# bytedance/ps-lite

Hardware: AMD Instinct MI355X
Metric: push+pull GB/s per worker + p50 round-trip µs, 1 MB & 64 MB, at 1/2/4/8 GPUs (higher is better)
Workload: dtype fp32; 1 GPU; model=dense push+pull (ps-lite test_benchmark PUSH_PULL), global_batch=128, seq_len=67108864, parallelism=byteps-joint x1 (worker+server per GPU), mode=dense, msg_bytes=67108864, batch_keys=False, overlap=True, op=assign

## Files before the change

### csrc/customer.cc

```cpp
#include "customer.h"

#include <chrono>

#include "postoffice.h"

namespace xps {

Customer::Customer(int app_id, int customer_id, RecvHandle handle, Postoffice* po)
    : app_id_(app_id), customer_id_(customer_id), handle_(std::move(handle)), po_(po) {
  po_->AddCustomer(this);
  thread_ = std::thread([this] { Receiving(); });
}

Customer::~Customer() {
  po_->RemoveCustomer(this);
  Message term;
  term.meta.control.cmd = Control::TERMINATE;
  queue_.Push(std::move(term));
  if (thread_.joinable()) thread_.join();
}

int Customer::NewRequest(int recver) {
  std::lock_guard<std::mutex> lk(mu_);
  int expected = recver >= 8 ? 1 : static_cast<int>(po_->GetNodeIDs(recver).size());
  tracker_.emplace_back();
  tracker_.back().expected = expected;
  return static_cast<int>(tracker_.size()) - 1;
}

Customer::Slot* Customer::GetSlot(int ts) {
  std::lock_guard<std::mutex> lk(mu_);
  XPS_CHECK_LT(static_cast<size_t>(ts), tracker_.size());
  return &tracker_[ts];
}

void Customer::WaitRequest(int ts) {
  Slot* s = GetSlot(ts);
  auto deadline = std::chrono::steady_clock::now() + std::chrono::microseconds(150);
  while (s->received.load(std::memory_order_acquire) < s->expected) {
    if (std::chrono::steady_clock::now() >= deadline) break;
  }
  if (s->received.load(std::memory_order_acquire) >= s->expected) return;
  static const int timeout_s = Environment::Get()->GetInt("XPS_WAIT_TIMEOUT_S", 0);
  std::unique_lock<std::mutex> lk(mu_);
  auto done = [s] { return s->received.load(std::memory_order_acquire) >= s->expected; };
  if (timeout_s <= 0) {
    cv_.wait(lk, done);
    return;
  }
  if (!cv_.wait_for(lk, std::chrono::seconds(timeout_s), done)) {
    XPS_LOG(Fatal) << "request ts=" << ts << " (app " << app_id_ << ") got "
                   << s->received.load() << "/" << s->expected << " responses after "
                   << timeout_s << " s — responder dead? (XPS_WAIT_TIMEOUT_S)";
  }
}

bool Customer::IsFinished(int ts) {
  Slot* s = GetSlot(ts);
  return s->received.load(std::memory_order_acquire) >= s->expected;
}

int Customer::NumResponse(int ts) {
  return GetSlot(ts)->received.load(std::memory_order_acquire);
}

void Customer::AddResponse(int ts, int num) {
  Slot* s = GetSlot(ts);
  int got = s->received.fetch_add(num, std::memory_order_acq_rel) + num;
  if (got >= s->expected) {
    std::lock_guard<std::mutex> lk(mu_);
    cv_.notify_all();
  }
}

thread_local int g_in_handler = 0;

bool InCustomerHandler() { return g_in_handler > 0; }

void Customer::RunHandle(Message& msg) {
  g_in_handler++;
  handle_(msg);
  g_in_handler--;
  if (!msg.meta.request) AddResponse(msg.meta.timestamp, 1);
}

void Customer::ProcessInline(Message& msg) {
  XPS_STAGE(customer_process);
  std::lock_guard<std::mutex> lk(handle_mu_);
  RunHandle(msg);
}

void Customer::Receiving() {
  while (true) {
    Message msg;
    queue_.WaitAndPop(&msg);
    if (msg.meta.control.cmd == Control::TERMINATE) break;
    std::lock_guard<std::mutex> lk(handle_mu_);
    RunHandle(msg);
  }
}

}
```

### csrc/customer.h

```cpp
#pragma once

#include <atomic>
#include <condition_variable>
#include <deque>
#include <functional>
#include <mutex>
#include <thread>
#include <utility>

#include "message.h"
#include "queue.h"

namespace xps {

class Postoffice;

bool InCustomerHandler();

class Customer {
 public:
  using RecvHandle = std::function<void(const Message&)>;

  Customer(int app_id, int customer_id, RecvHandle handle, Postoffice* po);
  ~Customer();
  Customer(const Customer&) = delete;

  int app_id() const { return app_id_; }
  int customer_id() const { return customer_id_; }

  int NewRequest(int recver);
  void WaitRequest(int ts);
  int NumResponse(int ts);
  void AddResponse(int ts, int num = 1);
  bool IsFinished(int ts);

  void Accept(Message msg) { queue_.Push(std::move(msg)); }

  void ProcessInline(Message& msg);

 private:
  struct Slot {
    int expected = 0;
    std::atomic<int> received{0};
  };

  void Receiving();
  void RunHandle(Message& msg);
  Slot* GetSlot(int ts);

  int app_id_;
  int customer_id_;
  RecvHandle handle_;
  Postoffice* po_;
  ThreadsafeQueue<Message> queue_;
  std::thread thread_;
  std::mutex handle_mu_;
  std::mutex mu_;
  std::condition_variable cv_;
  std::deque<Slot> tracker_;
};

}
```

### csrc/gpu_plane.cc

```cpp
#include "gpu_plane.h"

#include <fcntl.h>
#include <hip/hip_runtime.h>
#include <semaphore.h>
#include <sys/prctl.h>
#include <time.h>
#include <unistd.h>

#include <cstring>

#include "hip_pool.h"
#include "host_par.h"
#include "host_pool.h"
#include "kernels.h"
#include "postoffice.h"
#include "wire.h"

namespace xps {

static const size_t kInlineMax = 4096;

#define XPS_HIP_CHECK(cmd)                                                            \
  do {                                                                                \
    hipError_t e_ = (cmd);                                                            \
    XPS_CHECK(e_ == hipSuccess) << "HIP error: " << hipGetErrorString(e_) << " in " #cmd; \
  } while (0)

std::atomic<uint64_t> g_zero_copy_recv{0};
std::atomic<uint64_t> g_fused_assign{0};

bool FusedAssignEnabled() {
  static const bool on = Environment::Get()->GetInt("XPS_FUSED_ASSIGN", 1) != 0;
  return on;
}

std::atomic<uint64_t> g_fused_launches{0};

bool CoalesceEnabled() {
  static const bool on = Environment::Get()->GetInt("XPS_COALESCE", 1) != 0;
  return on;
}

namespace {
struct CoTicket {
  const void* plane = nullptr;
  int peer = 0;
  std::shared_ptr<void> cev;
};
thread_local CoTicket t_co_ticket;

int64_t NowUs() {
  struct timespec ts;
  clock_gettime(CLOCK_MONOTONIC, &ts);
  return static_cast<int64_t>(ts.tv_sec) * 1000000 + ts.tv_nsec / 1000;
}
const int64_t kHoldQuietUs = 2000;
const size_t kCoBusyBytes = 16u << 20;

std::mutex g_map_mu;
struct HandleKey {
  char h[kIpcHandleBytes];
  bool operator==(const HandleKey& o) const { return memcmp(h, o.h, kIpcHandleBytes) == 0; }
};
struct HandleHash {
  size_t operator()(const HandleKey& k) const {
    size_t v = 1469598103934665603ull;
    for (char c : k.h) {
      v ^= static_cast<unsigned char>(c);
      v *= 1099511628211ull;
    }
    return v;
  }
};
std::unordered_map<HandleKey, void*, HandleHash> g_mapped;

class IpcOpenLock {
 public:
  IpcOpenLock() {
    sem_ = sem_open("/xps_ipc_open_lock", O_CREAT, 0600, 1);
  }
  void Lock() {
    if (sem_ == SEM_FAILED) return;
    struct timespec ts;
    clock_gettime(CLOCK_REALTIME, &ts);
    ts.tv_sec += 60;
    if (sem_timedwait(sem_, &ts) != 0) {
      XPS_LOG(Warning) << "ipc-open lock timeout; proceeding unlocked";
      timed_out_ = true;
    }
  }
  void Unlock() {
    if (sem_ != SEM_FAILED && !timed_out_) sem_post(sem_);
    timed_out_ = false;
  }

 private:
  sem_t* sem_ = SEM_FAILED;
  bool timed_out_ = false;
};
IpcOpenLock g_ipc_lock;
}

GpuPlane::GpuPlane(Postoffice* po, int device) : po_(po), device_(device) {
  my_host_hash_ = HostHash();
  inline_deliver_ = Environment::Get()->GetInt("XPS_INLINE_HANDLER", 1) != 0;
  lanes_ = Environment::Get()->GetInt("XPS_STREAMS_PER_PEER", 2);
  if (lanes_ < 1) lanes_ = 1;
  if (lanes_ > 2) lanes_ = 2;
  co_hold_ = Environment::Get()->GetInt("XPS_COALESCE_HOLD", 0) != 0;
  int cap_mb = Environment::Get()->GetInt("XPS_COALESCE_CAP_MB", 1024);
  co_byte_cap_ = static_cast<size_t>(cap_mb < 1 ? 1 : cap_mb) << 20;
}

GpuPlane::~GpuPlane() { Stop(); }

void GpuPlane::FillSelf(Node* self) {
  static std::once_flag gc_once;
  std::call_once(gc_once, [] { HostShmPool::GcStaleSegments(); });
  self->dev_id = device_;
  auto* pool = HbmPool::Get();
  if (device_ >= 0 && pool->initialized()) {
    self->pool_capacity = pool->capacity();
    self->pool_slab_bytes = pool->slab_bytes();
    self->pool_handles.resize(pool->slab_count());
    for (size_t i = 0; i < pool->slab_count(); ++i) {
      memcpy(self->pool_handles[i].data(), pool->slab_handle(i), kIpcHandleBytes);
    }
  }
  auto* hpool = HostShmPool::Get();
  hpool->Init(self->shm_uid);
  self->host_pool_uid = hpool->uid();
  self->host_pool_capacity = hpool->capacity();
  if (!started_) {
    auto* env = Environment::Get();
    if (!env->GetInt("XPS_PROBE_NO_RING", 0)) {
      XPS_CHECK(in_ring_.Create(self->shm_uid)) << "cannot create shm ring";
    }
    started_ = true;
    if (!env->GetInt("XPS_PROBE_NO_POLL", 0)) {
      poll_running_ = true;
      poll_thread_ = std::thread([this] { RingPollLoop(); });
    }
    if (device_ >= 0 && !env->GetInt("XPS_PROBE_NO_COMP", 0)) {
      comp_thread_ = std::thread([this] { CompletionLoop(); });
    }
  }
}

void GpuPlane::Stop() {
  if (stop_.exchange(true)) return;
  PrintStageStats(device_ >= 0 ? "gpu plane" : "host plane");
  if (poll_thread_.joinable()) poll_thread_.join();
  if (comp_thread_.joinable()) comp_thread_.join();
  {
    std::lock_guard<std::mutex> lk(local_mu_);
    for (auto& lm : local_q_) po_->van()->Deliver(std::move(lm.first));
    local_q_.clear();
  }
  if (device_ >= 0) {
    std::vector<Peer*> all;
    {
      std::shared_lock<std::shared_timed_mutex> lk(peers_mu_);
      for (auto& kv : peers_) all.push_back(kv.second.get());
    }
// ... 187 lines not shown
          hipError_t e2 = hipMemcpy(probe, base, sizeof(probe), hipMemcpyDeviceToHost);
          if (e2 != hipSuccess) {
            XPS_LOG(Warning) << "peer " << p->node.id << " slab " << i
                             << " mapped but unreadable (" << hipGetErrorString(e2)
                             << ") — peer stays on the TCP path";
            base = nullptr;
          }
        }
        g_mapped[key] = base;
      }
    }
    if (!base) {
      std::lock_guard<std::mutex> lk(p->mu);
      p->slab_bases.clear();
      return false;
    }
    bases.push_back(base);
  }
  std::lock_guard<std::mutex> lk(p->mu);
  p->slab_bases = std::move(bases);
  return !p->slab_bases.empty();
}

char* GpuPlane::ResolvePeer(Peer* p, uint64_t global_off, uint64_t len) {
  if (!ImportPeerSlabs(p)) return nullptr;
  uint64_t slab_bytes = p->node.pool_slab_bytes;
  if (slab_bytes == 0) return nullptr;
  size_t idx = static_cast<size_t>(global_off / slab_bytes);
  uint64_t local = global_off % slab_bytes;
  std::lock_guard<std::mutex> lk(p->mu);
  if (idx >= p->slab_bases.size() || len > slab_bytes - local) {
    XPS_LOG(Warning) << "peer offset out of bounds: off=" << global_off << " len=" << len
                     << " slab=" << idx;
    return nullptr;
  }
  return static_cast<char*>(p->slab_bases[idx]) + local;
}

hipStream_t GpuPlane::StreamLane(int node_id, int lane) {
  if (lane >= lanes_) lane = lanes_ - 1;
  Peer* p = GetPeer(node_id);
  if (lane == 0) CoFlush(p);
  return RawLane(p, lane);
}

bool GpuPlane::LanesSplit(int node_id) {
  return lanes_ >= 2 && GetPeer(node_id)->node.dev_id != device_;
}


void GpuPlane::CoLaunchLocked(Peer* p) {
  Coalescer& co = p->co;
  if (co.n == 0) return;
  hipStream_t stream = RawLane(p, 0);
  XPS_HIP_CHECK(hipSetDevice(device_));
  if (co.n == 1) {
    const kern::Seg2& s = co.segs[0];
    kern::DenseAssign2(s.dst0, s.dst1, s.src, s.nbytes, stream);
  } else {
    kern::BatchedAssign2(co.segs, co.n, stream);
  }
  g_fused_launches.fetch_add(1, std::memory_order_relaxed);
  hipEvent_t ev = GetEvent();
  XPS_HIP_CHECK(hipEventRecord(ev, stream));
  co.open->bytes = co.bytes;
  co.open->ev.store(ev, std::memory_order_release);
  co.inflight.push_back(std::move(co.open));
  co.open.reset();
  co.n = 0;
  co.bytes = 0;
  co.n_open.store(0, std::memory_order_release);
}

bool GpuPlane::CoBusyLocked(Peer* p) {
  CoPruneLocked(p);
  size_t bytes = 0;
  for (auto& f : p->co.inflight) bytes += f->bytes;
  return p->co.inflight.size() >= 2 && bytes >= kCoBusyBytes;
}

void GpuPlane::CoPruneLocked(Peer* p) {
  auto& fl = p->co.inflight;
  while (!fl.empty()) {
    CoEvent* f = fl.front().get();
    if (!f->done.load(std::memory_order_acquire) &&
        hipEventQuery(f->ev.load(std::memory_order_acquire)) != hipSuccess) {
      break;
    }
    fl.pop_front();
  }
}

void GpuPlane::CoFlush(Peer* p) {
  if (p->co.n_open.load(std::memory_order_acquire) == 0) return;
  std::lock_guard<std::mutex> lk(p->co.mu);
  CoLaunchLocked(p);
}

std::shared_ptr<GpuPlane::CoEvent> GpuPlane::CoAppend(Peer* p, const kern::Seg2& seg) {
  if (!CoalesceEnabled()) return nullptr;
  Coalescer& co = p->co;
  std::lock_guard<std::mutex> lk(co.mu);
  kern::Admit a = kern::CoalesceAdmit(co.segs, co.n, seg);
  if (a != kern::Admit::kAdmit) CoLaunchLocked(p);
  if (a == kern::Admit::kReject) return nullptr;
  if (!co.open) co.open = std::make_shared<CoEvent>(this);
  std::shared_ptr<CoEvent> cev = co.open;
  co.segs[co.n++] = seg;
  co.bytes += seg.nbytes;
  co.n_open.store(co.n, std::memory_order_release);
  if (co.n >= kern::kMaxBatch || co.bytes >= co_byte_cap_) {
    CoLaunchLocked(p);
  } else if (co_hold_) {
    co.last_append_us = NowUs();
  } else {
    if (!CoBusyLocked(p)) CoLaunchLocked(p);
  }
  return cev;
}

bool GpuPlane::CoFrontUnlaunched(Peer* p, const std::shared_ptr<CoEvent>& cev) {
  Coalescer& co = p->co;
  std::lock_guard<std::mutex> lk(co.mu);
  if (co.open != cev) return true;
  if (co_hold_ && NowUs() - co.last_append_us < kHoldQuietUs) return false;
  CoLaunchLocked(p);
  return true;
}

void GpuPlane::CoRetired(Peer* p) {
  Coalescer& co = p->co;
  std::lock_guard<std::mutex> lk(co.mu);
  bool busy = CoBusyLocked(p);
  if (!co_hold_ && !busy) CoLaunchLocked(p);
}

bool GpuPlane::CoalesceAppend(int peer_id, const kern::Seg2& seg) {
  if (device_ < 0) return false;
  std::shared_ptr<CoEvent> cev = CoAppend(GetPeer(peer_id), seg);
  if (!cev) return false;
  t_co_ticket.plane = this;
  t_co_ticket.peer = peer_id;
  t_co_ticket.cev = std::move(cev);
  return true;
}

std::shared_ptr<GpuPlane::CoEvent> GpuPlane::TakeTicket(int peer_id) {
  if (!t_co_ticket.cev || t_co_ticket.plane != this || t_co_ticket.peer != peer_id) {
    return nullptr;
  }
  auto cev = std::static_pointer_cast<CoEvent>(t_co_ticket.cev);
  t_co_ticket.cev.reset();
  return cev;
}

void GpuPlane::CoalesceEnd(int peer_id) {
  if (!t_co_ticket.cev) return;
  t_co_ticket.cev.reset();
  CoFlush(GetPeer(peer_id));
}

hipStream_t GpuPlane::RawLane(Peer* p, int lane) {
  hipStream_t s = p->streams[lane].load(std::memory_order_acquire);
  if (s) return s;
  std::lock_guard<std::mutex> lk(p->mu);
  s = p->streams[lane].load(std::memory_order_relaxed);
  if (!s) {
    XPS_HIP_CHECK(hipSetDevice(device_));
    XPS_HIP_CHECK(hipStreamCreateWithFlags(&s, hipStreamNonBlocking));
    p->streams[lane].store(s, std::memory_order_release);
  }
  return s;
}

hipStream_t GpuPlane::StreamForPeer(int node_id) { return StreamLane(node_id, 0); }

hipStream_t GpuPlane::PullStreamForPeer(int node_id) {
  Peer* p = GetPeer(node_id);
  if (lanes_ < 2 || p->node.dev_id == device_) return StreamLane(node_id, 0);
  CoFlush(p);
  return StreamLane(node_id, 1);
}

std::vector<std::tuple<int, int64_t, int64_t>> GpuPlane::PeerBytes() {
  std::vector<std::tuple<int, int64_t, int64_t>> out;
  std::shared_lock<std::shared_timed_mutex> lk(peers_mu_);
  for (auto& kv : peers_) {
    int64_t tx = kv.second->tx_bytes.load(std::memory_order_relaxed);
    int64_t rx = kv.second->rx_bytes.load(std::memory_order_relaxed);
    if (tx || rx) out.emplace_back(kv.first, tx, rx);
  }
  return out;
// ... 137 lines not shown
bool GpuPlane::LocalPullRead(int peer_id, void* dst, uint64_t entry_off, size_t len,
                             Message resp) {
  if (device_ < 0 || !started_ || stop_.load()) return false;
  Peer* p = GetPeer(peer_id);
  char* src = ResolvePeer(p, entry_off, len);
  if (!src) return false;
  XPS_STAGE(local_pull_read);
  hipStream_t stream;
  if (Postoffice* elpo = LocalPeer(p)) {
    auto* rplane = dynamic_cast<GpuPlane*>(elpo->van() ? elpo->van()->plane() : nullptr);
    if (!rplane) return false;
    static const bool queue_req = Environment::Get()->GetInt("XPS_LOCAL_QUEUE_REQ", 0) != 0;
    if (!inline_deliver_ || queue_req) return false;
    stream = rplane->StreamForPeer(po_->node_id());
  } else {
    stream = StreamForPeer(peer_id);
  }
  XPS_HIP_CHECK(hipSetDevice(device_));
  kern::DenseAssign(dst, src, len, stream);
  g_zero_copy_recv.fetch_add(1, std::memory_order_relaxed);
  hipEvent_t ev = GetEvent();
  XPS_HIP_CHECK(hipEventRecord(ev, stream));
  int64_t bytes = static_cast<int64_t>(len) + 64;
  {
    std::lock_guard<std::mutex> lk(pend_mu_);
    pending_[peer_id].push_back(Pending{ev, peer_id, std::string(), std::move(resp), Message(),
                                        bytes, po_});
  }
  pending_count_.fetch_add(1);
  p->rx_bytes.fetch_add(bytes, std::memory_order_relaxed);
  return true;
}

bool GpuPlane::EntryPushPull(Message& msg, Peer* p, int64_t* bytes_out) {
  if (!FusedAssignEnabled()) return false;
  if (!(msg.meta.option & kOptPullAddr) || (msg.meta.option & kOptHostAddr)) return false;
  static const bool local_one_sided =
      Environment::Get()->GetInt("XPS_LOCAL_ONE_SIDED", 0) != 0;
  Postoffice* elpo = LocalPeer(p);
  GpuPlane* rplane =
      elpo ? dynamic_cast<GpuPlane*>(elpo->van() ? elpo->van()->plane() : nullptr) : nullptr;
  bool can = elpo ? (local_one_sided && rplane != nullptr) : EnsureRing(p);
  if (!can) return false;
  SArray<char> vals = msg.data[1];
  size_t len = vals.size();
  if (len == 0) return false;
  char* entry = ResolvePeer(p, msg.meta.entry_addr, len);
  char* dst = static_cast<char*>(HbmPool::Get()->PtrOf(msg.meta.addr, len));
  if (!entry || !dst || !kern::Disjoint3(entry, dst, vals.data(), len)) return false;
  XPS_STAGE(entry_push_pull);
  std::shared_ptr<CoEvent> cev;
  static const bool co_one_sided =
      Environment::Get()->GetInt("XPS_COALESCE_ONE_SIDED", 0) != 0;
  if (!elpo && co_one_sided) cev = CoAppend(p, kern::Seg2{entry, dst, vals.data(), len});
  hipStream_t stream = nullptr;
  if (!cev) {
    stream = elpo ? rplane->StreamForPeer(po_->node_id()) : StreamForPeer(p->node.id);
    XPS_HIP_CHECK(hipSetDevice(device_));
    kern::DenseAssign2(entry, dst, vals.data(), len, stream);
    g_fused_launches.fetch_add(1, std::memory_order_relaxed);
  }
  g_fused_assign.fetch_add(1, std::memory_order_relaxed);
  g_zero_copy_recv.fetch_add(1, std::memory_order_relaxed);
  Message meta_msg;
  meta_msg.meta = msg.meta;
  meta_msg.meta.option |= kOptInPlace;
  meta_msg.meta.val_len = static_cast<int64_t>(len);
  meta_msg.meta.data_type.clear();
  for (size_t i = 0; i < msg.data.size(); ++i) {
    if (i == 1 || msg.data[i].on_device()) continue;
    meta_msg.data.push_back(msg.data[i]);
    meta_msg.meta.data_type.push_back(msg.meta.data_type[i]);
  }
  int64_t bytes = 64 + static_cast<int64_t>(len);
  Message keepalive;
  keepalive.data.push_back(vals);
  std::string payload;
  if (!elpo) {
    std::vector<char> br(meta_msg.data.size(), 0);
    XPS_CHECK(Serialize(meta_msg, br, &payload));
  }
  hipEvent_t ev = nullptr;
  if (!cev) {
    ev = GetEvent();
    XPS_HIP_CHECK(hipEventRecord(ev, stream));
  }
  {
    std::lock_guard<std::mutex> lk(pend_mu_);
    pending_[p->node.id].push_back(Pending{ev, p->node.id, std::move(payload),
                                           std::move(meta_msg), std::move(keepalive), bytes,
                                           elpo, std::move(cev)});
  }
  pending_count_.fetch_add(1);
  p->tx_bytes.fetch_add(bytes, std::memory_order_relaxed);
  *bytes_out = bytes;
  return true;
}

void GpuPlane::EnqueueLocal(Message msg, int64_t bytes) {
  {
    std::lock_guard<std::mutex> lk(local_mu_);
    local_q_.emplace_back(std::move(msg), bytes);
  }
  local_count_.fetch_add(1, std::memory_order_release);
}

int64_t GpuPlane::SendLocal(Message& msg, Peer* p, Postoffice* lpo) {
// ... 263 lines not shown
    if (msg.data[i].on_device()) {
      by_ref[i] = 1;
      ref_bytes += msg.data[i].size();
      if (i == 1) msg.meta.option |= kOptValsByRef;
    } else if (msg.data[i].size() > kInlineMax) {
      by_ref[i] = 2;
      ref_bytes += msg.data[i].size();
    }
  }
  std::string payload;
  if (!Serialize(msg, by_ref, &payload)) {
    if (response && device_ >= 0) (void)hipStreamSynchronize(StreamForPeer(peer_node.id));
    return -1;
  }
  int64_t bytes = static_cast<int64_t>(payload.size()) + ref_bytes;
  bool kernel_less_ack = KernelLessAck(msg);
  if (response && device_ >= 0 && !kernel_less_ack) {
    hipStream_t stream = (msg.meta.option & kOptPullLane) ? PullStreamForPeer(peer_node.id)
                                                          : StreamForPeer(peer_node.id);
    Message resend = msg;
    DeferSendInternal(p, peer_node.id, stream, std::move(resend), Message(), std::move(payload),
                      bytes);
  } else {
    auto ring = RingOf(p);
    if (!ring || !ring->Push(payload.data(), static_cast<uint32_t>(payload.size()))) return -1;
    XPS_VLOG(3) << "plane send done -> " << peer_node.id;
  }
  p->tx_bytes.fetch_add(bytes, std::memory_order_relaxed);
  return bytes;
}

void GpuPlane::DeferSendInternal(Peer* p, int peer_id, hipStream_t stream, Message resend,
                                 Message keepalive, std::string payload, int64_t bytes) {
  XPS_STAGE(defer_queue);
  XPS_CHECK_GE(device_, 0) << "deferred sends are a GPU-plane feature";
  hipEvent_t ev = GetEvent();
  XPS_HIP_CHECK(hipSetDevice(device_));
  XPS_HIP_CHECK(hipEventRecord(ev, stream));
  {
    std::lock_guard<std::mutex> lk(pend_mu_);
    pending_[peer_id].push_back(Pending{ev, peer_id, std::move(payload), std::move(resend),
                                        std::move(keepalive), bytes});
  }
  pending_count_.fetch_add(1);
  XPS_VLOG(3) << "deferred send queued -> " << peer_id;
}

void GpuPlane::CompletionLoop() {
  XPS_HIP_CHECK(hipSetDevice(device_));
  prctl(PR_SET_TIMERSLACK, 1000);
  const int kSpin = Environment::Get()->GetInt("XPS_POLL_SPIN", 200000);
  int idle = 0;
  std::vector<int> ids;
  while (!stop_.load()) {
    bool did = false;
    if (pending_count_.load(std::memory_order_acquire) > 0) {
      ids.clear();
      {
        std::lock_guard<std::mutex> lk(pend_mu_);
        for (auto& kv : pending_) {
          if (!kv.second.empty()) ids.push_back(kv.first);
        }
      }
      for (int id : ids) {
        while (!stop_.load()) {
          hipEvent_t front_ev = nullptr;
          std::shared_ptr<CoEvent> cev;
          {
            std::lock_guard<std::mutex> lk(pend_mu_);
            auto& dq = pending_[id];
            if (dq.empty()) break;
            front_ev = dq.front().ev;
            cev = dq.front().cev;
          }
          bool retired = false;
          if (cev) {
            front_ev = cev->ev.load(std::memory_order_acquire);
            if (!front_ev) {
              if (!CoFrontUnlaunched(GetPeer(id), cev)) break;
              continue;
            }
          }
          if (!cev || !cev->done.load(std::memory_order_acquire)) {
            hipError_t e = hipEventQuery(front_ev);
            if (e == hipErrorNotReady) break;
            XPS_CHECK(e == hipSuccess) << "hipEventQuery: " << hipGetErrorString(e);
            if (cev) {
              cev->done.store(true, std::memory_order_release);
              retired = true;
            }
          }
          XPS_STAGE(defer_release);
          if (retired) CoRetired(GetPeer(id));
          Pending front;
          {
            std::lock_guard<std::mutex> lk(pend_mu_);
            auto& dq = pending_[id];
            front = std::move(dq.front());
            dq.pop_front();
          }
          pending_count_.fetch_sub(1);
          if (front.local_po) {
            DeliverLocal(front.local_po, front.resend, front.bytes);
            if (front.ev) PutEvent(front.ev);
            did = true;
            continue;
          }
          Peer* peer = GetPeer(front.peer_id);
          auto ring = peer ? RingOf(peer) : nullptr;
          bool sent = ring && ring->Push(front.payload.data(),
                                         static_cast<uint32_t>(front.payload.size()));
          if (sent) {
            XPS_VLOG(3) << "deferred send done -> " << front.peer_id;
          } else {
            XPS_LOG(Warning) << "deferred plane send failed -> " << front.peer_id
                             << "; falling back to TCP";
            if (po_->van()->SendOverTcp(front.resend, front.peer_id) < 0) {
              XPS_LOG(Warning) << "TCP fallback to " << front.peer_id
                               << " failed too (peer dead?)";
            }
          }
          if (front.ev) PutEvent(front.ev);
          did = true;
        }
      }
    }
    if (did) {
      idle = 0;
    } else if (++idle > kSpin) {
      usleep(20);
    }
  }
}

void GpuPlane::RingPollLoop() {
  if (device_ >= 0) XPS_HIP_CHECK(hipSetDevice(device_));
  prctl(PR_SET_TIMERSLACK, 1000);
  const int kSpin = Environment::Get()->GetInt("XPS_POLL_SPIN", 200000);
  std::vector<char> buf(ShmRing::MaxPayload());
  int idle = 0;
  std::deque<std::pair<Message, int64_t>> local;
  while (!stop_.load()) {
    if (local_count_.load(std::memory_order_acquire) > 0) {
      {
        std::lock_guard<std::mutex> lk(local_mu_);
        local.swap(local_q_);
      }
      local_count_.fetch_sub(static_cast<int>(local.size()));
      for (auto& lm : local) {
        XPS_STAGE(local_handle);
        po_->van()->recv_bytes_ += lm.second;
        for (auto& d : lm.first.data) {
          if (d.size() && (d.on_device() || d.size() > kInlineMax)) {
            g_zero_copy_recv.fetch_add(1, std::memory_order_relaxed);
          }
        }
        if (inline_deliver_) {
          po_->van()->DeliverInline(lm.first);
        } else {
          po_->van()->Deliver(std::move(lm.first));
        }
      }
      idle = 0;
      local.clear();
    }
    uint32_t n = in_ring_.Pop(buf.data());
    if (n == 0) {
      if (++idle > kSpin) usleep(20);
      continue;
    }
    idle = 0;
    XPS_STAGE(ring_handle);
    ByteReader r(buf.data(), n);
    uint64_t meta_len = r.U64();
    Message msg;
    {
// ... 67 lines not shown
```

### csrc/gpu_plane.h

```cpp
#pragma once

#include <hip/hip_runtime.h>

#include <atomic>
#include <deque>
#include <memory>
#include <shared_mutex>
#include <thread>
#include <tuple>
#include <unordered_map>
#include <vector>

#include "kernels.h"
#include "shm_ring.h"
#include "van.h"

namespace xps {

extern std::atomic<uint64_t> g_zero_copy_recv;
extern std::atomic<uint64_t> g_fused_assign;
bool FusedAssignEnabled();
extern std::atomic<uint64_t> g_fused_launches;
bool CoalesceEnabled();

class Postoffice;

class GpuPlane : public DataPlane {
 public:
  GpuPlane(Postoffice* po, int device);
  ~GpuPlane() override;

  void FillSelf(Node* self) override;
  void ImportPeers() override;
  bool CanSend(const Message& msg, const Node& peer) override;
  int64_t Send(Message& msg, const Node& peer) override;
  void OnPeer(const Node& peer) override;
  void Stop() override;

  hipStream_t StreamForPeer(int node_id);
  hipStream_t PullStreamForPeer(int node_id);
  int lanes() const { return lanes_; }
  bool LanesSplit(int node_id);

  bool CoalesceAppend(int peer_id, const kern::Seg2& seg);
  void CoalesceEnd(int peer_id);
  std::vector<std::tuple<int, int64_t, int64_t>> PeerBytes();
  int device() const { return device_; }

  bool LocalPullRead(int peer_id, void* dst, uint64_t entry_off, size_t len, Message resp);
  hipEvent_t GetEvent();
  void PutEvent(hipEvent_t ev);
  char* PeerDst(int peer_id, uint64_t global_off, uint64_t len) {
    return ResolvePeer(GetPeer(peer_id), global_off, len);
  }

 private:
  struct CoEvent {
    explicit CoEvent(GpuPlane* pl) : plane(pl) {}
    ~CoEvent() {
      if (hipEvent_t e = ev.load(std::memory_order_acquire)) plane->PutEvent(e);
    }
    GpuPlane* plane;
    std::atomic<hipEvent_t> ev{nullptr};
    std::atomic<bool> done{false};
    size_t bytes = 0;
  };
  struct Coalescer {
    std::mutex mu;
    kern::Seg2 segs[kern::kMaxBatch];
    int n = 0;
    std::atomic<int> n_open{0};
    size_t bytes = 0;
    std::shared_ptr<CoEvent> open;
    std::deque<std::shared_ptr<CoEvent>> inflight;
    int64_t last_append_us = 0;
  };

  struct Peer {
    Node node;
    Coalescer co;
    std::atomic<Postoffice*> local_po{nullptr};
    std::shared_ptr<ShmRing> ring;
    bool ring_tried = false;
    std::atomic<bool> ring_ok{false};
    std::vector<void*> slab_bases;
    bool pool_tried = false;
    std::atomic<hipStream_t> streams[2] = {{nullptr}, {nullptr}};
    std::atomic<int64_t> tx_bytes{0};
    std::atomic<int64_t> rx_bytes{0};
    std::mutex mu;
  };

  struct Pending {
    hipEvent_t ev;
    int peer_id;
    std::string payload;
    Message resend;
    Message keepalive;
    int64_t bytes;
    Postoffice* local_po = nullptr;
    std::shared_ptr<CoEvent> cev;
  };

  Peer* GetPeer(int id);
  Postoffice* LocalPeer(Peer* p);
  int64_t SendLocal(Message& msg, Peer* p, Postoffice* lpo);
  void DeliverLocal(Postoffice* lpo, Message& msg, int64_t bytes);
  void EnqueueLocal(Message msg, int64_t bytes);
  bool EnsureRing(Peer* p);
  std::shared_ptr<ShmRing> RingOf(Peer* p);
  bool ImportPeerSlabs(Peer* p);
  char* ResolvePeer(Peer* p, uint64_t global_off, uint64_t len);
  bool Serialize(const Message& msg, const std::vector<char>& by_ref, std::string* out);
  void RingPollLoop();
  void CompletionLoop();
  hipStream_t StreamLane(int node_id, int lane);
  hipStream_t RawLane(Peer* p, int lane);
  std::shared_ptr<CoEvent> CoAppend(Peer* p, const kern::Seg2& seg);
  void CoLaunchLocked(Peer* p);
  void CoPruneLocked(Peer* p);
  bool CoBusyLocked(Peer* p);
  void CoFlush(Peer* p);
  bool CoFrontUnlaunched(Peer* p, const std::shared_ptr<CoEvent>& cev);
  void CoRetired(Peer* p);
  std::shared_ptr<CoEvent> TakeTicket(int peer_id);
  bool EntryPushPull(Message& msg, Peer* p, int64_t* bytes_out);
  void DeferSendInternal(Peer* p, int peer_id, hipStream_t stream, Message resend,
                         Message keepalive, std::string payload, int64_t bytes);

  Postoffice* po_;
  int device_;
  int lanes_ = 2;
  bool co_hold_ = false;
  size_t co_byte_cap_ = 1ull << 30;
  uint64_t my_host_hash_;
  ShmRing in_ring_;
  bool started_ = false;
  bool inline_deliver_ = true;

  std::shared_timed_mutex peers_mu_;
  std::unordered_map<int, std::unique_ptr<Peer>> peers_;

  std::thread poll_thread_;
  std::thread comp_thread_;
  std::atomic<bool> stop_{false};

  std::mutex pend_mu_;
  std::unordered_map<int, std::deque<Pending>> pending_;
  std::atomic<int> pending_count_{0};

  std::mutex local_mu_;
  std::deque<std::pair<Message, int64_t>> local_q_;
  std::atomic<int> local_count_{0};
  bool poll_running_ = false;

  std::mutex ev_mu_;
  std::vector<hipEvent_t> event_pool_;
};

std::shared_ptr<DataPlane> CreateGpuPlane(Postoffice* po, int device);

}
```

### csrc/pybind.cc

```cpp
#include <pybind11/functional.h>
#include <pybind11/numpy.h>
#include <pybind11/pybind11.h>
#include <pybind11/stl.h>

#include <atomic>
#include <thread>

#include "gpu_plane.h"
#include "hip_pool.h"
#include "hip_util.h"
#include "host_pool.h"
#include "kernels.h"
#include "kv_app.h"
#include "kv_utils.h"
#include "mxfp8.h"
#include "ps.h"
#include "server_handlers.h"
#include "shm_ring.h"
#include "simple_app.h"
#include "tile_runs.h"
#include "van.h"
#include "wire.h"

namespace py = pybind11;
using namespace xps;

namespace {

struct PoolBuffer {
  SArray<char> arr;
  uintptr_t ptr() const { return reinterpret_cast<uintptr_t>(arr.data()); }
  size_t nbytes() const { return arr.size(); }
  int device() const { return arr.device(); }
  void copy_from(py::array src) {
    py::buffer_info info = src.request();
    size_t n = static_cast<size_t>(info.size) * info.itemsize;
    XPS_CHECK_LE(n, arr.size());
    if (arr.on_device()) {
      gpu::CopyHostToDevice(arr.data(), info.ptr, n, arr.device());
    } else {
      memcpy(arr.data(), info.ptr, n);
    }
  }
  py::array_t<float> to_numpy_f32() const {
    size_t n = arr.size() / sizeof(float);
    py::array_t<float> out(n);
    if (arr.on_device()) {
      gpu::CopyDeviceToHost(out.mutable_data(), arr.data(), n * sizeof(float));
    } else {
      memcpy(out.mutable_data(), arr.data(), n * sizeof(float));
    }
    return out;
  }
};

class PyKVWorker {
 public:
  PyKVWorker(int app_id, int customer_id, int instance_idx)
      : w_(app_id, customer_id, instance_idx) {}

// ... 49 lines not shown
    if (lens.size()) l.CopyFrom(lens.data(), lens.size());
    SArray<Key> kd;
    if (keys_dev_ptr) {
      kd = SArray<Key>(reinterpret_cast<Key*>(keys_dev_ptr), keys.size(), device);
    }
    py::gil_scoped_release rel;
    return w_.ZPushPull(k, v, out, l, cmd, [out]() { delete out; }, kd);
  }

  int ZPullPtr(py::array_t<uint64_t> keys, uintptr_t vals_ptr, size_t vals_bytes, int device,
               py::array_t<int> lens, int cmd, uintptr_t keys_dev_ptr) {
    SArray<Key> k;
    k.CopyFrom(keys.data(), keys.size());
    auto* v = new SArray<float>(reinterpret_cast<float*>(vals_ptr), vals_bytes / sizeof(float),
                                device);
    SArray<int>* l = nullptr;
    if (lens.size()) {
      l = new SArray<int>();
      l->CopyFrom(lens.data(), lens.size());
    }
    SArray<Key> kd;
    if (keys_dev_ptr) {
      kd = SArray<Key>(reinterpret_cast<Key*>(keys_dev_ptr), keys.size(), device);
    }
    py::gil_scoped_release rel;
    return w_.ZPull(k, v, l, cmd, [v, l]() {
      delete v;
      delete l;
    }, kd);
  }

  void Wait(int ts) {
    py::gil_scoped_release rel;
    w_.Wait(ts);
  }

  void RoundMixed(py::array_t<uint64_t> keys, const std::vector<uintptr_t>& push_ptrs,
                  const std::vector<uintptr_t>& pull_ptrs, const std::vector<size_t>& sizes,
                  int device, int cmd, bool overlap) {
    size_t nk = static_cast<size_t>(keys.size());
    XPS_CHECK_EQ(push_ptrs.size(), nk);
    std::vector<SArray<Key>> karrs(nk);
    for (size_t i = 0; i < nk; ++i) karrs[i] = SArray<Key>({keys.data()[i]});
    py::gil_scoped_release rel;
    std::vector<int> tss;
    tss.reserve(2 * nk);
    std::vector<std::unique_ptr<SArray<float>>> dsts;
    std::vector<int> pull_tss;
    auto issue_pull = [&](size_t i) {
      size_t n = sizes[i] / sizeof(float);
      dsts.emplace_back(new SArray<float>(reinterpret_cast<float*>(pull_ptrs[i]), n, device));
      return w_.ZPull(karrs[i], dsts.back().get(), nullptr, cmd);
    };
    for (size_t i = 0; i < nk; ++i) {
      size_t n = sizes[i] / sizeof(float);
      SArray<int> lens(1);
      lens[0] = static_cast<int>(n);
      SArray<float> v(reinterpret_cast<float*>(push_ptrs[i]), n, device);
      if (overlap && !pull_ptrs.empty() && device >= 0 && cmd != kCmdSum &&
          push_ptrs[i] != pull_ptrs[i] && FusedAssignEnabled() &&
          w_.HasEntry(keys.data()[i], sizes[i])) {
        dsts.emplace_back(new SArray<float>(reinterpret_cast<float*>(pull_ptrs[i]), n, device));
        tss.push_back(w_.ZPushPull(karrs[i], v, dsts.back().get(), lens, cmd));
        continue;
      }
      tss.push_back(w_.ZPush(karrs[i], v, lens, cmd));
      if (overlap && !pull_ptrs.empty()) tss.push_back(issue_pull(i));
    }
    if (!overlap && !pull_ptrs.empty()) {
      for (int ts : tss) w_.Wait(ts);
      tss.clear();
      for (size_t i = 0; i < nk; ++i) tss.push_back(issue_pull(i));
    }
    for (int ts : tss) w_.Wait(ts);
  }

  void Round(py::array_t<uint64_t> keys, const std::vector<uintptr_t>& ptrs, size_t nbytes,
             int device, int cmd, bool pull) {
    size_t nk = static_cast<size_t>(keys.size());
    XPS_CHECK_EQ(ptrs.size(), nk);
    size_t n = nbytes / sizeof(float);
    std::vector<SArray<Key>> karrs(nk);
    for (size_t i = 0; i < nk; ++i) karrs[i] = SArray<Key>({keys.data()[i]});
    SArray<int> lens(1);
    lens[0] = static_cast<int>(n);
    py::gil_scoped_release rel;
    std::vector<int> tss(nk);
    std::vector<std::unique_ptr<SArray<float>>> dsts;
    for (size_t i = 0; i < nk; ++i) {
      if (pull) {
        dsts.emplace_back(new SArray<float>(reinterpret_cast<float*>(ptrs[i]), n, device));
        tss[i] = w_.ZPull(karrs[i], dsts.back().get(), nullptr, cmd);
      } else {
        SArray<float> v(reinterpret_cast<float*>(ptrs[i]), n, device);
        tss[i] = w_.ZPush(karrs[i], v, lens, cmd);
      }
    }
    for (int ts : tss) w_.Wait(ts);
  }

 private:
  KVWorker<float> w_;
};

class PyKVServer {
 public:
  explicit PyKVServer(int app_id, int instance_idx) : s_(app_id, instance_idx) {}

  void SetDefaultHandle() {
    auto h = std::make_shared<KVServerDefaultHandle<float>>();
    default_ = h;
    s_.set_request_handle([h](const KVMeta& m, const KVPairs<float>& kvs, KVServer<float>* srv) {
      (*h)(m, kvs, srv);
    });
  }

  void SetReduceHandle(int num_workers) {
    auto h = std::make_shared<KVServerReduceHandle<float>>(num_workers);
    reduce_ = h;
    s_.set_request_handle([h](const KVMeta& m, const KVPairs<float>& kvs, KVServer<float>* srv) {
      (*h)(m, kvs, srv);
    });
  }

  void RegisterEntry(uint64_t key, uintptr_t ptr, size_t nbytes, int device) {
    XPS_CHECK(dense_) << "register_entry needs set_gpu_dense_handle first";
    dense_->RegisterEntry(key, reinterpret_cast<void*>(ptr), nbytes, device);
  }

  void SaveCheckpoint(const std::string& path) {
    py::gil_scoped_release rel;
    if (dense_) {
      dense_->Save(path);
    } else if (sparse_) {
      sparse_->Save(path);
    } else if (default_ || reduce_) {
      FILE* f = fopen(path.c_str(), "wb");
      XPS_CHECK(f) << "cannot open checkpoint " << path;
      uint64_t n = default_ ? default_->store.size() : reduce_->store.size();
      fwrite(&n, 8, 1, f);
      auto write_one = [f](uint64_t key, const float* data, uint64_t len) {
        fwrite(&key, 8, 1, f);
        fwrite(&len, 8, 1, f);
        fwrite(data, 1, len, f);
      };
      if (default_) {
        for (auto& kv : default_->store) {
          write_one(kv.first, kv.second.data(), kv.second.size() * sizeof(float));
        }
      } else {
        for (auto& kv : reduce_->store) {
          write_one(kv.first, kv.second.buf.data(), kv.second.buf.size() * sizeof(float));
        }
      }
// ... 276 lines not shown
      .def("set_reduce_handle", &PyKVServer::SetReduceHandle, py::arg("num_workers"))
      .def("set_gpu_dense_handle", &PyKVServer::SetGpuDenseHandle, py::arg("mode") = "assign",
           py::arg("dtype") = "f32")
      .def("set_gpu_sparse_handle", &PyKVServer::SetGpuSparseHandle, py::arg("rows"),
           py::arg("row_len"), py::arg("accumulate") = true, py::arg("key_shift") = 0)
      .def("register_entry", &PyKVServer::RegisterEntry, py::arg("key"), py::arg("ptr"),
           py::arg("nbytes"), py::arg("device") = 0)
      .def("sparse_table_ptr", &PyKVServer::SparseTablePtr)
      .def("save_checkpoint", &PyKVServer::SaveCheckpoint)
      .def("load_checkpoint", &PyKVServer::LoadCheckpoint)
      .def("set_python_handle", &PyKVServer::SetPythonHandle);

  m.def("zero_copy_recv_count", []() { return g_zero_copy_recv.load(); });
  m.def("fused_assign_count", []() { return g_fused_assign.load(); });
  m.def("fused_assign_launches", []() { return g_fused_launches.load(); });
  m.def("mxfp8_launches", []() { return g_mx_launches.load(); });
  m.def("mxfp8_packed_nbytes", [](size_t n) { return mx::MxPackedBytes(n); }, py::arg("n"));
  m.def("mxfp8_quantize_host",
        [](py::array_t<float, py::array::c_style | py::array::forcecast> src) {
          size_t n = static_cast<size_t>(src.size());
          py::array_t<uint8_t> out(mx::MxPackedBytes(n));
          mx::MxQuantizeHost(src.data(), n, out.mutable_data());
          return out;
        },
        py::arg("src"));
  m.def("mxfp8_dequantize_host",
        [](py::array_t<uint8_t, py::array::c_style | py::array::forcecast> packed, size_t n,
           float alpha) {
          if (static_cast<size_t>(packed.size()) < mx::MxPackedBytes(n)) {
            throw std::invalid_argument("mxfp8_dequantize_host: packed is shorter than n elements");
          }
          py::array_t<float> out(n);
          mx::MxDequantizeHost(packed.data(), n, out.mutable_data(), alpha);
          return out;
        },
        py::arg("packed"), py::arg("n"), py::arg("alpha") = 1.0f);
  m.def("coalesce_admit",
        [](const std::vector<std::tuple<uintptr_t, uintptr_t, uintptr_t, size_t>>& open,
           const std::tuple<uintptr_t, uintptr_t, uintptr_t, size_t>& seg) {
          auto conv = [](const std::tuple<uintptr_t, uintptr_t, uintptr_t, size_t>& t) {
            return kern::Seg2{reinterpret_cast<void*>(std::get<0>(t)),
                              reinterpret_cast<void*>(std::get<1>(t)),
                              reinterpret_cast<const void*>(std::get<2>(t)), std::get<3>(t)};
          };
          std::vector<kern::Seg2> segs;
          for (auto& t : open) segs.push_back(conv(t));
          switch (kern::CoalesceAdmit(segs.data(), static_cast<int>(segs.size()), conv(seg))) {
            case kern::Admit::kAdmit: return "admit";
            case kern::Admit::kFlushFirst: return "flush";
            default: return "reject";
          }
        },
        py::arg("open"), py::arg("seg"));
  m.def("tile_runs",
        [](const std::vector<unsigned long long>& chunk_counts,
           unsigned long long chunks_per_block, unsigned long long block_index) {
          if (chunks_per_block == 0) throw std::invalid_argument("tile_runs: empty tile");
          std::vector<unsigned long long> prefix(chunk_counts.size() + 1, 0);
          for (size_t i = 0; i < chunk_counts.size(); ++i) {
            if (chunk_counts[i] == 0) throw std::invalid_argument("tile_runs: empty segment");
            prefix[i + 1] = prefix[i] + chunk_counts[i];
          }
          int n = static_cast<int>(chunk_counts.size());
          std::vector<std::tuple<int, unsigned long long, unsigned long long>> out;
          kern::TileRunIter it = kern::TileRunsBegin(prefix.data(), n, chunks_per_block,
                                                     block_index);
          kern::TileRun run;
          while (kern::TileRunsNext(prefix.data(), &it, &run)) {
            out.emplace_back(run.seg, run.lo, run.hi);
          }
          return out;
        },
        py::arg("chunk_counts"), py::arg("chunks_per_block"), py::arg("block_index"));

  m.def("plane_peer_bytes", [](const std::string& role, int idx) {
    py::dict out;
    auto* po = GetPO(role, idx);
    auto* plane = po->van() ? dynamic_cast<GpuPlane*>(po->van()->plane()) : nullptr;
    if (plane) {
      for (auto& t : plane->PeerBytes()) {
        out[py::int_(std::get<0>(t))] = py::make_tuple(std::get<1>(t), std::get<2>(t));
      }
    }
    return out;
  }, py::arg("role") = "worker", py::arg("idx") = 0);

  m.def("_order_nodes", [](std::vector<std::tuple<std::string, std::string, int>> in) {
    std::vector<Node> nodes;
    for (auto& t : in) {
      Node n;
      n.role = std::get<0>(t) == "worker" ? Node::WORKER : Node::SERVER;
      n.hostname = std::get<1>(t);
      n.port = std::get<2>(t);
      nodes.push_back(n);
    }
    auto less = NodeRankOrder(nodes);
    std::sort(nodes.begin(), nodes.end(), less);
    std::vector<std::tuple<std::string, std::string, int>> out;
    for (auto& n : nodes) {
      out.emplace_back(n.role == Node::WORKER ? "worker" : "server", n.hostname, n.port);
    }
    return out;
  });

  m.def("_host_pool_init_for_test", [](uint64_t uid, size_t bytes) {
    HostShmPool::Get()->Init(uid, bytes);
// ... 375 lines not shown
```

Before: 3828 GB/s.

## Cork coalesced copies within a push/pull batch and flush on wait

Adds a thread-local cork scope around the batch issue loop so coalesced segment appends are held until a byte floor (default 64 MB) is reached or the scope ends or a wait begins, instead of launching each one when the stream is idle. The launch policy is centralised in a pure CorkLaunch function. The completion loop now remembers peers whose front is blocked and spins without re-scanning, and it releases all pending entries that share one coalesced event at once. Customer only notifies the condition variable when a waiter is registered. These aim to cut kernel launches and per-message lock and notify overhead, at the cost of added latency for partially filled batches and more complex state.

After: 3810 GB/s. About the same (-0.5%).

```diff
diff --git a/csrc/cork.h b/csrc/cork.h
--- /dev/null
+++ b/csrc/cork.h
@@ -0,0 +1,15 @@
+#pragma once
+
+namespace xps {
+
+class CorkScope {
+ public:
+  CorkScope();
+  ~CorkScope();
+  CorkScope(const CorkScope&) = delete;
+  CorkScope& operator=(const CorkScope&) = delete;
+};
+
+void CorkFlushThisThread();
+
+}
diff --git a/csrc/cork_policy.h b/csrc/cork_policy.h
--- /dev/null
+++ b/csrc/cork_policy.h
@@ -0,0 +1,61 @@
+#pragma once
+
+#include <cstddef>
+#include <cstdint>
+
+namespace xps {
+namespace kern {
+
+enum class CorkAsk {
+  kAppend,
+  kFront,
+  kRetired,
+  kRelease,
+};
+
+struct CorkState {
+  bool corked = false;
+  int n_open = 0;
+  size_t open_bytes = 0;
+  size_t floor_bytes = 0;
+  size_t byte_cap = 0;
+  int max_batch = 0;
+  bool busy = false;
+  bool hold = false;
+  int64_t quiet_us = 0;
+  int64_t backstop_us = 0;
+  CorkAsk who = CorkAsk::kAppend;
+};
+
+static const size_t kCorkFloorMaxBytes = 64u << 20;
+
+inline size_t CorkFloorBytes(long long mb) {
+  if (mb <= 0) return 0;
+  size_t b = static_cast<size_t>(mb) << 20;
+  return b > kCorkFloorMaxBytes ? kCorkFloorMaxBytes : b;
+}
+
+inline bool CorkLaunch(const CorkState& s) {
+  if (s.n_open <= 0) return false;
+  if (s.n_open >= s.max_batch || s.open_bytes >= s.byte_cap) return true;
+  if (s.who == CorkAsk::kRelease) return true;
+  bool quiet = s.quiet_us >= s.backstop_us;
+  if (s.hold) {
+    return s.who == CorkAsk::kFront && quiet;
+  }
+  if (s.corked && s.floor_bytes > 0 && s.open_bytes < s.floor_bytes) {
+    return s.who == CorkAsk::kFront && quiet;
+  }
+  if (s.who == CorkAsk::kFront) return true;
+  return !s.busy;
+}
+
+inline bool CorkBusyMatters(CorkState s) {
+  s.busy = false;
+  bool idle = CorkLaunch(s);
+  s.busy = true;
+  return idle != CorkLaunch(s);
+}
+
+}
+}
diff --git a/csrc/customer.cc b/csrc/customer.cc
--- a/csrc/customer.cc
+++ b/csrc/customer.cc
@@ -2,6 +2,7 @@
 
 #include <chrono>
 
+#include "cork.h"
 #include "postoffice.h"
 
 namespace xps {
@@ -35,6 +36,7 @@
 }
 
 void Customer::WaitRequest(int ts) {
+  CorkFlushThisThread();
   Slot* s = GetSlot(ts);
   auto deadline = std::chrono::steady_clock::now() + std::chrono::microseconds(150);
   while (s->received.load(std::memory_order_acquire) < s->expected) {
@@ -43,7 +45,12 @@
   if (s->received.load(std::memory_order_acquire) >= s->expected) return;
   static const int timeout_s = Environment::Get()->GetInt("XPS_WAIT_TIMEOUT_S", 0);
   std::unique_lock<std::mutex> lk(mu_);
-  auto done = [s] { return s->received.load(std::memory_order_acquire) >= s->expected; };
+  s->waiters.fetch_add(1);
+  struct Unregister {
+    Slot* s;
+    ~Unregister() { s->waiters.fetch_sub(1); }
+  } unregister{s};
+  auto done = [s] { return s->received.load() >= s->expected; };
   if (timeout_s <= 0) {
     cv_.wait(lk, done);
     return;
@@ -66,8 +73,8 @@
 
 void Customer::AddResponse(int ts, int num) {
   Slot* s = GetSlot(ts);
-  int got = s->received.fetch_add(num, std::memory_order_acq_rel) + num;
-  if (got >= s->expected) {
+  int got = s->received.fetch_add(num) + num;
+  if (got >= s->expected && s->waiters.load() > 0) {
     std::lock_guard<std::mutex> lk(mu_);
     cv_.notify_all();
   }
diff --git a/csrc/customer.h b/csrc/customer.h
--- a/csrc/customer.h
+++ b/csrc/customer.h
@@ -42,6 +42,7 @@
   struct Slot {
     int expected = 0;
     std::atomic<int> received{0};
+    std::atomic<int> waiters{0};
   };
 
   void Receiving();
diff --git a/csrc/gpu_plane.cc b/csrc/gpu_plane.cc
--- a/csrc/gpu_plane.cc
+++ b/csrc/gpu_plane.cc
@@ -9,6 +9,7 @@
 
 #include <cstring>
 
+#include "cork.h"
 #include "hip_pool.h"
 #include "host_par.h"
 #include "host_pool.h"
@@ -48,6 +49,12 @@
   std::shared_ptr<void> cev;
 };
 thread_local CoTicket t_co_ticket;
+
+struct ThreadCork {
+  int depth = 0;
+  std::vector<std::pair<GpuPlane*, void*>> open;
+};
+thread_local ThreadCork t_cork;
 
 int64_t NowUs() {
   struct timespec ts;
@@ -110,6 +117,7 @@
   co_hold_ = Environment::Get()->GetInt("XPS_COALESCE_HOLD", 0) != 0;
   int cap_mb = Environment::Get()->GetInt("XPS_COALESCE_CAP_MB", 1024);
   co_byte_cap_ = static_cast<size_t>(cap_mb < 1 ? 1 : cap_mb) << 20;
+  cork_floor_ = kern::CorkFloorBytes(Environment::Get()->GetInt("XPS_CORK_MB", 64));
 }
 
 GpuPlane::~GpuPlane() { Stop(); }
@@ -403,6 +411,7 @@
 void GpuPlane::CoLaunchLocked(Peer* p) {
   Coalescer& co = p->co;
   if (co.n == 0) return;
+  XPS_STAGE(co_launch);
   hipStream_t stream = RawLane(p, 0);
   XPS_HIP_CHECK(hipSetDevice(device_));
   if (co.n == 1) {
@@ -420,7 +429,37 @@
   co.open.reset();
   co.n = 0;
   co.bytes = 0;
+  co.corked = false;
+  co.front_waits.store(false, std::memory_order_release);
   co.n_open.store(0, std::memory_order_release);
+}
+
+kern::CorkState GpuPlane::CoStateLocked(Peer* p, bool corked, kern::CorkAsk who) {
+  Coalescer& co = p->co;
+  kern::CorkState s;
+  s.corked = corked;
+  s.n_open = co.n;
+  s.open_bytes = co.bytes;
+  s.floor_bytes = cork_floor_;
+  s.byte_cap = co_byte_cap_;
+  s.max_batch = kern::kMaxBatch;
+  s.hold = co_hold_;
+  s.backstop_us = kHoldQuietUs;
+  s.who = who;
+  return s;
+}
+
+bool GpuPlane::CoDecideLocked(Peer* p, bool corked, kern::CorkAsk who, const bool* busy_known) {
+  kern::CorkState s = CoStateLocked(p, corked, who);
+  if (who == kern::CorkAsk::kFront) {
+    s.quiet_us = NowUs() - p->co.last_append_us.load(std::memory_order_acquire);
+  }
+  if (busy_known) {
+    s.busy = *busy_known;
+  } else if (kern::CorkBusyMatters(s)) {
+    s.busy = CoBusyLocked(p);
+  }
+  return kern::CorkLaunch(s);
 }
 
 bool GpuPlane::CoBusyLocked(Peer* p) {
@@ -445,11 +484,30 @@
 void GpuPlane::CoFlush(Peer* p) {
   if (p->co.n_open.load(std::memory_order_acquire) == 0) return;
   std::lock_guard<std::mutex> lk(p->co.mu);
-  CoLaunchLocked(p);
-}
-
-std::shared_ptr<GpuPlane::CoEvent> GpuPlane::CoAppend(Peer* p, const kern::Seg2& seg) {
+  if (CoDecideLocked(p, p->co.corked, kern::CorkAsk::kRelease)) CoLaunchLocked(p);
+}
+
+void GpuPlane::CorkRelease(void* co_peer) { CoFlush(static_cast<Peer*>(co_peer)); }
+
+CorkScope::CorkScope() { ++t_cork.depth; }
+
+CorkScope::~CorkScope() {
+  if (--t_cork.depth == 0) CorkFlushThisThread();
+}
+
+void CorkFlushThisThread() {
+  if (t_cork.open.empty()) return;
+  XPS_STAGE(cork_flush);
+  std::vector<std::pair<GpuPlane*, void*>> open;
+  open.swap(t_cork.open);
+  for (auto& o : open) o.first->CorkRelease(o.second);
+}
+
+std::shared_ptr<GpuPlane::CoEvent> GpuPlane::CoAppend(Peer* p, const kern::Seg2& seg,
+                                                      bool may_cork) {
   if (!CoalesceEnabled()) return nullptr;
+  XPS_STAGE(co_append);
+  bool corked = may_cork && cork_floor_ > 0 && t_cork.depth > 0;
   Coalescer& co = p->co;
   std::lock_guard<std::mutex> lk(co.mu);
   kern::Admit a = kern::CoalesceAdmit(co.segs, co.n, seg);
@@ -460,21 +518,36 @@
   co.segs[co.n++] = seg;
   co.bytes += seg.nbytes;
   co.n_open.store(co.n, std::memory_order_release);
-  if (co.n >= kern::kMaxBatch || co.bytes >= co_byte_cap_) {
+  if (CoDecideLocked(p, corked, kern::CorkAsk::kAppend)) {
     CoLaunchLocked(p);
-  } else if (co_hold_) {
-    co.last_append_us = NowUs();
-  } else {
-    if (!CoBusyLocked(p)) CoLaunchLocked(p);
+    return cev;
+  }
+  co.corked = corked;
+  if (co_hold_ || corked) co.last_append_us.store(NowUs(), std::memory_order_release);
+  kern::CorkState front = CoStateLocked(p, corked, kern::CorkAsk::kFront);
+  bool waits = !kern::CorkLaunch(front);
+  co.front_waits.store(waits, std::memory_order_release);
+  if (corked && waits) {
+    bool known = false;
+    for (auto& o : t_cork.open) known = known || o.second == p;
+    if (!known) t_cork.open.emplace_back(this, p);
   }
   return cev;
+}
+
+bool GpuPlane::CoStillHeld(Peer* p, const std::shared_ptr<CoEvent>& cev) {
+  Coalescer& co = p->co;
+  return !cev->ev.load(std::memory_order_acquire) &&
+         co.front_waits.load(std::memory_order_acquire) &&
+         NowUs() - co.last_append_us.load(std::memory_order_acquire) < kHoldQuietUs;
 }
 
 bool GpuPlane::CoFrontUnlaunched(Peer* p, const std::shared_ptr<CoEvent>& cev) {
   Coalescer& co = p->co;
+  if (CoStillHeld(p, cev)) return false;
   std::lock_guard<std::mutex> lk(co.mu);
   if (co.open != cev) return true;
-  if (co_hold_ && NowUs() - co.last_append_us < kHoldQuietUs) return false;
+  if (!CoDecideLocked(p, co.corked, kern::CorkAsk::kFront)) return false;
   CoLaunchLocked(p);
   return true;
 }
@@ -483,12 +556,12 @@
   Coalescer& co = p->co;
   std::lock_guard<std::mutex> lk(co.mu);
   bool busy = CoBusyLocked(p);
-  if (!co_hold_ && !busy) CoLaunchLocked(p);
+  if (CoDecideLocked(p, co.corked, kern::CorkAsk::kRetired, &busy)) CoLaunchLocked(p);
 }
 
 bool GpuPlane::CoalesceAppend(int peer_id, const kern::Seg2& seg) {
   if (device_ < 0) return false;
-  std::shared_ptr<CoEvent> cev = CoAppend(GetPeer(peer_id), seg);
+  std::shared_ptr<CoEvent> cev = CoAppend(GetPeer(peer_id), seg, true);
   if (!cev) return false;
   t_co_ticket.plane = this;
   t_co_ticket.peer = peer_id;
@@ -732,7 +805,9 @@
   std::shared_ptr<CoEvent> cev;
   static const bool co_one_sided =
       Environment::Get()->GetInt("XPS_COALESCE_ONE_SIDED", 0) != 0;
-  if (!elpo && co_one_sided) cev = CoAppend(p, kern::Seg2{entry, dst, vals.data(), len});
+  if (!elpo && co_one_sided) {
+    cev = CoAppend(p, kern::Seg2{entry, dst, vals.data(), len}, false);
+  }
   hipStream_t stream = nullptr;
   if (!cev) {
     stream = elpo ? rplane->StreamForPeer(po_->node_id()) : StreamForPeer(p->node.id);
@@ -1102,9 +1177,30 @@
   const int kSpin = Environment::Get()->GetInt("XPS_POLL_SPIN", 200000);
   int idle = 0;
   std::vector<int> ids;
+  std::vector<Pending> rel;
+  struct Blocked {
+    std::shared_ptr<CoEvent> cev;
+    Peer* peer;
+    hipEvent_t ev;
+    bool Still(GpuPlane* pl) const {
+      hipEvent_t e = cev ? cev->ev.load(std::memory_order_acquire) : ev;
+      if (!e) return pl->CoStillHeld(peer, cev);
+      if (cev && cev->done.load(std::memory_order_acquire)) return false;
+      return hipEventQuery(e) == hipErrorNotReady;
+    }
+  };
+  std::unordered_map<int, Blocked> blocked;
   while (!stop_.load()) {
     bool did = false;
     if (pending_count_.load(std::memory_order_acquire) > 0) {
+      if (!blocked.empty() && blocked.size() == ids.size()) {
+        int seen = pending_count_.load(std::memory_order_acquire);
+        bool held = true;
+        while (held && !stop_.load() &&
+               pending_count_.load(std::memory_order_acquire) == seen) {
+          for (auto& b : blocked) held = held && b.second.Still(this);
+        }
+      }
       ids.clear();
       {
         std::lock_guard<std::mutex> lk(pend_mu_);
@@ -1113,6 +1209,11 @@
         }
       }
       for (int id : ids) {
+        auto b = blocked.find(id);
+        if (b != blocked.end()) {
+          if (b->second.Still(this)) continue;
+          blocked.erase(b);
+        }
         while (!stop_.load()) {
           hipEvent_t front_ev = nullptr;
           std::shared_ptr<CoEvent> cev;
@@ -1127,13 +1228,20 @@
           if (cev) {
             front_ev = cev->ev.load(std::memory_order_acquire);
             if (!front_ev) {
-              if (!CoFrontUnlaunched(GetPeer(id), cev)) break;
+              Peer* fp = GetPeer(id);
+              if (!CoFrontUnlaunched(fp, cev)) {
+                blocked[id] = Blocked{cev, fp, nullptr};
+                break;
+              }
               continue;
             }
           }
           if (!cev || !cev->done.load(std::memory_order_acquire)) {
             hipError_t e = hipEventQuery(front_ev);
-            if (e == hipErrorNotReady) break;
+            if (e == hipErrorNotReady) {
+              blocked[id] = Blocked{cev, nullptr, front_ev};
+              break;
+            }
             XPS_CHECK(e == hipSuccess) << "hipEventQuery: " << hipGetErrorString(e);
             if (cev) {
               cev->done.store(true, std::memory_order_release);
@@ -1142,36 +1250,41 @@
           }
           XPS_STAGE(defer_release);
           if (retired) CoRetired(GetPeer(id));
-          Pending front;
+          rel.clear();
           {
             std::lock_guard<std::mutex> lk(pend_mu_);
             auto& dq = pending_[id];
-            front = std::move(dq.front());
-            dq.pop_front();
+            do {
+              rel.push_back(std::move(dq.front()));
+              dq.pop_front();
+            } while (cev && !dq.empty() && dq.front().cev == cev);
           }
-          pending_count_.fetch_sub(1);
-          if (front.local_po) {
-            DeliverLocal(front.local_po, front.resend, front.bytes);
+          pending_count_.fetch_sub(static_cast<int>(rel.size()));
+          did = true;
+          for (Pending& front : rel) {
+            if (front.local_po) {
+              XPS_STAGE(defer_deliver);
+              DeliverLocal(front.local_po, front.resend, front.bytes);
+              if (front.ev) PutEvent(front.ev);
+              continue;
+            }
+            Peer* peer = GetPeer(front.peer_id);
+            auto ring = peer ? RingOf(peer) : nullptr;
+            bool sent = ring && ring->Push(front.payload.data(),
+                                           static_cast<uint32_t>(front.payload.size()));
+            if (sent) {
+              XPS_VLOG(3) << "deferred send done -> " << front.peer_id;
+            } else {
+              XPS_LOG(Warning) << "deferred plane send failed -> " << front.peer_id
+                               << "; falling back to TCP";
+              if (po_->van()->SendOverTcp(front.resend, front.peer_id) < 0) {
+                XPS_LOG(Warning) << "TCP fallback to " << front.peer_id
+                                 << " failed too (peer dead?)";
+              }
+            }
             if (front.ev) PutEvent(front.ev);
-            did = true;
-            continue;
           }
-          Peer* peer = GetPeer(front.peer_id);
-          auto ring = peer ? RingOf(peer) : nullptr;
-          bool sent = ring && ring->Push(front.payload.data(),
-                                         static_cast<uint32_t>(front.payload.size()));
-          if (sent) {
-            XPS_VLOG(3) << "deferred send done -> " << front.peer_id;
-          } else {
-            XPS_LOG(Warning) << "deferred plane send failed -> " << front.peer_id
-                             << "; falling back to TCP";
-            if (po_->van()->SendOverTcp(front.resend, front.peer_id) < 0) {
-              XPS_LOG(Warning) << "TCP fallback to " << front.peer_id
-                               << " failed too (peer dead?)";
-            }
-          }
-          if (front.ev) PutEvent(front.ev);
-          did = true;
+          rel.clear();
         }
       }
     }
diff --git a/csrc/gpu_plane.h b/csrc/gpu_plane.h
--- a/csrc/gpu_plane.h
+++ b/csrc/gpu_plane.h
@@ -11,6 +11,7 @@
 #include <unordered_map>
 #include <vector>
 
+#include "cork_policy.h"
 #include "kernels.h"
 #include "shm_ring.h"
 #include "van.h"
@@ -46,6 +47,7 @@
   void CoalesceEnd(int peer_id);
   std::vector<std::tuple<int, int64_t, int64_t>> PeerBytes();
   int device() const { return device_; }
+  void CorkRelease(void* co_peer);
 
   bool LocalPullRead(int peer_id, void* dst, uint64_t entry_off, size_t len, Message resp);
   hipEvent_t GetEvent();
@@ -73,7 +75,9 @@
     size_t bytes = 0;
     std::shared_ptr<CoEvent> open;
     std::deque<std::shared_ptr<CoEvent>> inflight;
-    int64_t last_append_us = 0;
+    std::atomic<int64_t> last_append_us{0};
+    bool corked = false;
+    std::atomic<bool> front_waits{false};
   };
 
   struct Peer {
@@ -116,12 +120,15 @@
   void CompletionLoop();
   hipStream_t StreamLane(int node_id, int lane);
   hipStream_t RawLane(Peer* p, int lane);
-  std::shared_ptr<CoEvent> CoAppend(Peer* p, const kern::Seg2& seg);
+  std::shared_ptr<CoEvent> CoAppend(Peer* p, const kern::Seg2& seg, bool may_cork);
   void CoLaunchLocked(Peer* p);
+  kern::CorkState CoStateLocked(Peer* p, bool corked, kern::CorkAsk who);
+  bool CoDecideLocked(Peer* p, bool corked, kern::CorkAsk who, const bool* busy_known = nullptr);
   void CoPruneLocked(Peer* p);
   bool CoBusyLocked(Peer* p);
   void CoFlush(Peer* p);
   bool CoFrontUnlaunched(Peer* p, const std::shared_ptr<CoEvent>& cev);
+  bool CoStillHeld(Peer* p, const std::shared_ptr<CoEvent>& cev);
   void CoRetired(Peer* p);
   std::shared_ptr<CoEvent> TakeTicket(int peer_id);
   bool EntryPushPull(Message& msg, Peer* p, int64_t* bytes_out);
@@ -133,6 +140,7 @@
   int lanes_ = 2;
   bool co_hold_ = false;
   size_t co_byte_cap_ = 1ull << 30;
+  size_t cork_floor_ = 64u << 20;
   uint64_t my_host_hash_;
   ShmRing in_ring_;
   bool started_ = false;
diff --git a/csrc/pybind.cc b/csrc/pybind.cc
--- a/csrc/pybind.cc
+++ b/csrc/pybind.cc
@@ -6,6 +6,8 @@
 #include <atomic>
 #include <thread>
 
+#include "cork.h"
+#include "cork_policy.h"
 #include "gpu_plane.h"
 #include "hip_pool.h"
 #include "hip_util.h"
@@ -161,6 +163,7 @@
       dsts.emplace_back(new SArray<float>(reinterpret_cast<float*>(pull_ptrs[i]), n, device));
       return w_.ZPull(karrs[i], dsts.back().get(), nullptr, cmd);
     };
+    std::unique_ptr<CorkScope> cork(new CorkScope());
     for (size_t i = 0; i < nk; ++i) {
       size_t n = sizes[i] / sizeof(float);
       SArray<int> lens(1);
@@ -176,12 +179,13 @@
       tss.push_back(w_.ZPush(karrs[i], v, lens, cmd));
       if (overlap && !pull_ptrs.empty()) tss.push_back(issue_pull(i));
     }
+    cork.reset();
     if (!overlap && !pull_ptrs.empty()) {
-      for (int ts : tss) w_.Wait(ts);
+      WaitAll(tss);
       tss.clear();
       for (size_t i = 0; i < nk; ++i) tss.push_back(issue_pull(i));
     }
-    for (int ts : tss) w_.Wait(ts);
+    WaitAll(tss);
   }
 
   void Round(py::array_t<uint64_t> keys, const std::vector<uintptr_t>& ptrs, size_t nbytes,
@@ -205,10 +209,15 @@
         tss[i] = w_.ZPush(karrs[i], v, lens, cmd);
       }
     }
+    WaitAll(tss);
+  }
+
+ private:
+  void WaitAll(const std::vector<int>& tss) {
+    if (!tss.empty()) w_.Wait(tss.back());
     for (int ts : tss) w_.Wait(ts);
   }
 
- private:
   KVWorker<float> w_;
 };
 
@@ -591,6 +600,39 @@
           }
         },
         py::arg("open"), py::arg("seg"));
+  m.def("cork_launch",
+        [](bool corked, int n_open, size_t open_bytes, size_t floor_bytes, size_t byte_cap,
+           bool busy, bool hold, long long quiet_us, const std::string& who, int max_batch,
+           long long backstop_us) {
+          kern::CorkState s;
+          s.corked = corked;
+          s.n_open = n_open;
+          s.open_bytes = open_bytes;
+          s.floor_bytes = floor_bytes;
+          s.byte_cap = byte_cap;
+          s.max_batch = max_batch;
+          s.busy = busy;
+          s.hold = hold;
+          s.quiet_us = quiet_us;
+          s.backstop_us = backstop_us;
+          if (who == "append") {
+            s.who = kern::CorkAsk::kAppend;
+          } else if (who == "front") {
+            s.who = kern::CorkAsk::kFront;
+          } else if (who == "retired") {
+            s.who = kern::CorkAsk::kRetired;
+          } else if (who == "release") {
+            s.who = kern::CorkAsk::kRelease;
+          } else {
+            throw std::invalid_argument("cork_launch: who is append, front, retired or release");
+          }
+          return kern::CorkLaunch(s);
+        },
+        py::arg("corked"), py::arg("n_open"), py::arg("open_bytes"), py::arg("floor_bytes"),
+        py::arg("byte_cap") = size_t(1) << 30, py::arg("busy") = false, py::arg("hold") = false,
+        py::arg("quiet_us") = 0, py::arg("who") = "append",
+        py::arg("max_batch") = static_cast<int>(kern::kMaxBatch), py::arg("backstop_us") = 2000);
+  m.def("cork_floor_bytes", [](long long mb) { return kern::CorkFloorBytes(mb); }, py::arg("mb"));
   m.def("tile_runs",
         [](const std::vector<unsigned long long>& chunk_counts,
            unsigned long long chunks_per_block, unsigned long long block_index) {
```
